# Mine268/CS-ViT

Measured on NVIDIA B200. Metric: images/sec Swin-B spatial fwd @224^2 bs256, higher is better.
Workload: dtype fp16

## Files before the change

### cs-vit_b200/csrc/mlp_fused.cu

```cuda
#include <cstdio>
#include <cstdlib>
#include <type_traits>

#include "errors.h"
#include "gemm.cuh"
#include "rowops.cuh"

namespace csvit {

constexpr uint32_t kUnit = 128 * 128;

template <int C>
struct MlpCfg {
  static constexpr int KB1 = C / 64;
  static constexpr int N2 = C / 128;
  static constexpr int NCH = 4 * C / 128;
  static constexpr int WSTAGES = 4;
  static constexpr int STG_BUFS = C == 128 ? 2 : 1;
  static constexpr uint32_t A1_BYTES = KB1 * kUnit;
  static constexpr uint32_t A2_BYTES = 2 * 2 * kUnit;
  static constexpr uint32_t W_BYTES = WSTAGES * kUnit;
  static constexpr uint32_t STG_BYTES = STG_BUFS * kEpiWarps * kStageBufBytes;
  static constexpr size_t SMEM = 1024 + size_t(A1_BYTES) + A2_BYTES + W_BYTES + STG_BYTES + 512;
};

struct MlpParams {
  const float* b1;
  int M;
  long long* trace;
};
constexpr int kMlpTraceTiles = 8;
#ifdef CSVIT_MLP_TRACE_BUILD
#define MLP_STAMP(k) do { if (tr) tr[k] = clock64(); } while (0)
#else
#define MLP_STAMP(k) do { } while (0)
#endif

constexpr int kMlpThreadsSplit = 640;
template <int FMT, int C, bool SPLIT>
__global__ void __launch_bounds__(SPLIT ? kMlpThreadsSplit : kGemmThreads, 1)
mlp_fused_kernel(const __grid_constant__ CUtensorMap tmX, const __grid_constant__ CUtensorMap tmW1,
                 const __grid_constant__ CUtensorMap tmW2, const __grid_constant__ CUtensorMap tmR, MlpParams mp, EpiParams ep) {
  using Cfg = MlpCfg<C>;
  static_assert(!SPLIT || C == 128, "the second GEMM2 accumulator fits TMEM at C = 128 only");
  constexpr int KB1 = Cfg::KB1, N2 = Cfg::N2, NCH = Cfg::NCH, WS = Cfg::WSTAGES;
  extern __shared__ uint8_t smem_raw[];
  const uint32_t base = (smem_u32(smem_raw) + 1023u) & ~1023u;
  uint8_t* smem = smem_raw + (base - smem_u32(smem_raw));
  const uint32_t a1_off = 0, a2_off = Cfg::A1_BYTES, w_off = a2_off + Cfg::A2_BYTES, stg_off = w_off + Cfg::W_BYTES;
  uint64_t* bars = reinterpret_cast<uint64_t*>(smem + stg_off + Cfg::STG_BYTES);
  uint64_t* w_full = bars;
  uint64_t* w_empty = bars + WS;
  uint64_t* acc1_full = bars + 2 * WS;
  uint64_t* acc1_empty = acc1_full + 2;
  uint64_t* a2_full = acc1_full + 4;
  uint64_t* a2_empty = acc1_full + 6;
  uint64_t* a1_full = acc1_full + 8;
  uint64_t* a1_empty = acc1_full + 9;
  uint64_t* acc2_full = acc1_full + 10;
  uint64_t* acc2_empty = acc1_full + 12;
  uint32_t* tmem_slot = reinterpret_cast<uint32_t*>(acc1_full + 14);
  uint64_t* rbar = bars + 32;

  const int warp = threadIdx.x >> 5, lane = threadIdx.x & 31;
  const int num_tiles = (mp.M + kBM - 1) / kBM;

  if (warp == 0 && lane == 0) {
    prefetch_tmap(&tmX); prefetch_tmap(&tmW1); prefetch_tmap(&tmW2);
    if (ep.tma_f32) prefetch_tmap(&tmR);
    for (int i = 0; i < 2 * kEpiWarps; ++i) mbar_init(&rbar[i], 1);
    for (int s = 0; s < WS; ++s) { mbar_init(&w_full[s], 1); mbar_init(&w_empty[s], 1); }
    for (int b = 0; b < 2; ++b) {
      mbar_init(&acc1_full[b], 1); mbar_init(&acc1_empty[b], kEpiWarps);
      mbar_init(&a2_full[b], kEpiWarps); mbar_init(&a2_empty[b], 1);
    }
    mbar_init(a1_full, 1); mbar_init(a1_empty, 1);
    for (int b = 0; b < 2; ++b) { mbar_init(&acc2_full[b], 1); mbar_init(&acc2_empty[b], kEpiWarps); }
    fence_mbar_init();
  }
  if (warp == 1) tmem_alloc(tmem_slot, 512);
  tc_fence_before();
  __syncthreads();
  tc_fence_after();
  const uint32_t tmem_base = *tmem_slot;
  griddep_launch();
  griddep_wait();
  const uint32_t tm_acc2 = tmem_base + 256;
  constexpr int EW0 = SPLIT ? 4 : 2;
  if (warp < EW0) {
  if (SPLIT) asm volatile("setmaxnreg.dec.sync.aligned.u32 64;");
  if (warp == 0) {
    if (lane == 0) {
      int s = 0; uint32_t ph = 0;
      auto load_w = [&](const CUtensorMap* tm, int col, int row) {
        mbar_wait(&w_empty[s], ph ^ 1u);
        mbar_arrive_expect_tx(&w_full[s], kUnit);
        tma_load_2d(smem + w_off + size_t(s) * kUnit, tm, &w_full[s], col, row);
        if (++s == WS) { s = 0; ph ^= 1u; }
      };
      uint32_t it = 0;
      auto load_a1 = [&](int t, uint32_t i) {
        mbar_wait(a1_empty, (i & 1u) ^ 1u);
        mbar_arrive_expect_tx(a1_full, Cfg::A1_BYTES);
        for (int kb = 0; kb < KB1; ++kb) tma_load_2d(smem + a1_off + size_t(kb) * kUnit, &tmX, a1_full, kb * 64, t * kBM);
      };
      bool pre = false;
      for (int t = blockIdx.x; t < num_tiles; t += gridDim.x, ++it) {
        if (!pre) {
          load_a1(t, it);
          for (int kb = 0; kb < KB1; ++kb) load_w(&tmW1, kb * 64, 0);
        }
        pre = false;
        for (int j = 0; j < NCH; ++j) {
          if (j + 1 < NCH) {
            for (int kb = 0; kb < KB1; ++kb) load_w(&tmW1, kb * 64, (j + 1) * 128);
          } else if (SPLIT && t + int(gridDim.x) < num_tiles) {
            load_a1(t + int(gridDim.x), it + 1);
            for (int kb = 0; kb < KB1; ++kb) load_w(&tmW1, kb * 64, 0);
            pre = true;
          }
          for (int kb2 = 0; kb2 < 2; ++kb2)
            for (int n2 = 0; n2 < N2; ++n2) load_w(&tmW2, j * 128 + kb2 * 64, n2 * 128);
        }
      }
    }
  } else if (warp == 1) {
    {
      constexpr uint32_t idesc = make_idesc(uint32_t(FMT), kBM, 128);
      int s = 0; uint32_t ph = 0;
      auto mma_unit = [&](uint32_t a_addr, uint32_t d_tmem, bool first) {
        mbar_wait(&w_full[s], ph);
        tc_fence_after();
        if (fa_elect_one()) {
          const uint64_t adesc = make_sw128_kmajor_desc(a_addr);
          const uint64_t bdesc = make_sw128_kmajor_desc(base + w_off + uint32_t(s) * kUnit);
#pragma unroll
          for (int k = 0; k < 4; ++k)
            umma_ss<false>(d_tmem, adesc + uint64_t(2 * k), bdesc + uint64_t(2 * k), idesc, (first && k == 0) ? 0u : 1u);
          umma_commit(&w_empty[s]);
        }
        __syncwarp();
        if (++s == WS) { s = 0; ph ^= 1u; }
      };
      uint32_t it = 0;
      uint32_t use[2] = {0, 0};
      auto gemm1 = [&](int j) {
        const int b = j & 1;
        mbar_wait(&acc1_empty[b], (use[b] & 1u) ^ 1u);
        tc_fence_after();
        for (int kb = 0; kb < KB1; ++kb) mma_unit(base + a1_off + uint32_t(kb) * kUnit, tmem_base + uint32_t(b * 128), kb == 0);
        if (fa_elect_one()) umma_commit(&acc1_full[b]);
        __syncwarp();
      };
      bool pre = false;
      for (int t = blockIdx.x; t < num_tiles; t += gridDim.x, ++it) {
        if (!pre) {
          mbar_wait(a1_full, it & 1u);
          tc_fence_after();
          gemm1(0);
        }
        pre = false;
        for (int j = 0; j < NCH; ++j) {
          const int b = j & 1;
          if (j + 1 < NCH) {
            gemm1(j + 1);
            if (j + 2 == NCH) { if (fa_elect_one()) umma_commit(a1_empty); __syncwarp(); }
          } else if (SPLIT && t + int(gridDim.x) < num_tiles) {
            mbar_wait(a1_full, (it + 1) & 1u);
            tc_fence_after();
            gemm1(0);
            pre = true;
          }
          mbar_wait(&a2_full[b], use[b] & 1u);
          tc_fence_after();
          const uint32_t ab = SPLIT ? (it & 1u) : 0u;
          if (j == 0) { mbar_wait(&acc2_empty[ab], ((SPLIT ? it >> 1 : it) & 1u) ^ 1u); tc_fence_after(); }
          for (int kb2 = 0; kb2 < 2; ++kb2)
            for (int n2 = 0; n2 < N2; ++n2)
              mma_unit(base + a2_off + uint32_t(b * 2 + kb2) * kUnit, tm_acc2 + ab * 128u + uint32_t(n2 * 128), j == 0 && kb2 == 0);
          if (fa_elect_one()) {
            umma_commit(&a2_empty[b]);
            if (j == NCH - 1) umma_commit(&acc2_full[ab]);
          }
          __syncwarp();
          ++use[b];
        }
      }
    }
  }
  } else if (SPLIT && warp >= 12) {
    asm volatile("setmaxnreg.dec.sync.aligned.u32 80;");
    const int e = warp - 12;
    const int quad = warp & 3;
    const int half = e >> 2;
    uint8_t* stg = smem + stg_off + e * Cfg::STG_BUFS * kStageBufBytes;
    uint32_t it = 0, rph = 0;
    for (int t = blockIdx.x; t < num_tiles; t += gridDim.x, ++it) {
      const uint32_t ab = it & 1u;
      const int row0 = t * kBM + quad * 32, colbase = half * 64;
      if (ep.red_add) {
        if (lane == 0) tma_store_wait_read0();
        __syncwarp();
      } else {
        tma_f32_prefetch<C>(ep, &tmR, stg, rbar + 2 * e, t, 0, quad, half, lane);
      }
      mbar_wait(&acc2_full[ab], (it >> 1) & 1u);
      tc_fence_after();
      const uint32_t t_addr = tm_acc2 + ab * 128u + (uint32_t(quad * 32) << 16) + uint32_t(colbase);
#pragma unroll 1
      for (int ci = 0; ci < 2; ++ci) {
        uint8_t* buf = stg + ci * kStageBufBytes;
        uint32_t rr[32];
        tmem_ld_32x32(t_addr + uint32_t(32 * ci), rr);
        tmem_ld_wait();
        if (row0 < ep.M && !ep.red_add) {
          mbar_wait(&rbar[2 * e + ci], (rph >> ci) & 1u);
          rph ^= (1u << ci);
        }
        const float4* b4 = reinterpret_cast<const float4*>(ep.bias + colbase + 32 * ci);
#pragma unroll
        for (int k = 0; k < 8; ++k) {
          float4* pp = reinterpret_cast<float4*>(buf + lane * 128 + ((k ^ (lane & 7)) << 4));
          const float4 bb = __ldg(b4 + k);
          float4 x0 = ep.red_add ? make_float4(0.f, 0.f, 0.f, 0.f) : *pp;
          x0.x += __uint_as_float(rr[4 * k]) + bb.x; x0.y += __uint_as_float(rr[4 * k + 1]) + bb.y;
          x0.z += __uint_as_float(rr[4 * k + 2]) + bb.z; x0.w += __uint_as_float(rr[4 * k + 3]) + bb.w;
          *pp = x0;
        }
        fence_proxy_async_smem();
        __syncwarp();
        if (lane == 0 && row0 < ep.M) {
          if (ep.red_add) tma_reduce_add_2d(&tmR, buf, colbase + 32 * ci, row0);
          else tma_store_2d(&tmR, buf, colbase + 32 * ci, row0);
          tma_store_commit();
        }
      }
      tc_fence_before();
      __syncwarp();
      if (lane == 0) mbar_arrive(&acc2_empty[ab]);
    }
  } else {
    if (SPLIT) asm volatile("setmaxnreg.inc.sync.aligned.u32 128;");
    const int e = warp - EW0;
    const int quad = warp & 3;
    const int half = e >> 2;
    const int r = quad * 32 + lane;
    const bool bf = FMT == 1;
    uint8_t* stg = smem + stg_off + e * Cfg::STG_BUFS * kStageBufBytes;
    uint32_t it = 0, rph = 0;
    uint32_t use[2] = {0, 0};
    for (int t = blockIdx.x; t < num_tiles; t += gridDim.x, ++it) {
      if (!SPLIT) {
        if (ep.tma_f32) tma_f32_prefetch<C>(ep, &tmR, stg, rbar + 2 * e, t, 0, quad, half, lane);
        else prefetch_resid_tile<C>(ep, t, 0, quad, half, lane);
      }
#ifdef CSVIT_MLP_TRACE_BUILD
      long long* tr = (mp.trace && blockIdx.x == 0 && e == 0 && lane == 0 && it < kMlpTraceTiles) ? mp.trace + it * 64 : nullptr;
#endif
      for (int j = 0; j < NCH; ++j) {
        const int b = j & 1;
        MLP_STAMP(4 * j);
        mbar_wait(&acc1_full[b], use[b] & 1u);
        tc_fence_after();
        MLP_STAMP(4 * j + 1);
        uint32_t rr0[32], rr1[32];
        {
          const uint32_t ta = tmem_base + (uint32_t(quad * 32) << 16) + uint32_t(b * 128 + half * 64);
          tmem_ld_32x32(ta, rr0);
          tmem_ld_32x32(ta + 32u, rr1);
          tmem_ld_wait();
        }
        tc_fence_before();
        __syncwarp();
        if (lane == 0) mbar_arrive(&acc1_empty[b]);
        uint32_t pk[32];
        epi_bias_gelu_pack32(mp.b1, bf, j * 128 + half * 64, rr0, pk);
        epi_bias_gelu_pack32(mp.b1, bf, j * 128 + half * 64 + 32, rr1, pk + 16);
        MLP_STAMP(4 * j + 2);
        mbar_wait(&a2_empty[b], (use[b] & 1u) ^ 1u);
        MLP_STAMP(4 * j + 3);
        uint8_t* dst = smem + a2_off + uint32_t(b * 2 + half) * kUnit + r * 128;
#pragma unroll
        for (int ci = 0; ci < 8; ++ci)
          *reinterpret_cast<uint4*>(dst + ((ci ^ (r & 7)) << 4)) = make_uint4(pk[4 * ci], pk[4 * ci + 1], pk[4 * ci + 2], pk[4 * ci + 3]);
        fence_proxy_async_smem();
        __syncwarp();
        if (lane == 0) mbar_arrive(&a2_full[b]);
        ++use[b];
      }
      MLP_STAMP(4 * NCH);
      if (!SPLIT) {
#ifdef CSVIT_MLP_TRACE_BUILD
        if (tr) { mbar_wait(&acc2_full[0], it & 1u); tr[4 * NCH + 1] = clock64(); }
#endif
        epilogue_tile<C>(ep, &tmR, stg, tm_acc2, &acc2_full[0], it & 1u, t, 0, quad, half, lane, 1, nullptr, &tmR, rbar + 2 * e, &rph, true);
        tc_fence_before();
        __syncwarp();
        if (lane == 0) mbar_arrive(&acc2_empty[0]);
      } else {
        MLP_STAMP(4 * NCH + 1);
      }
      MLP_STAMP(4 * NCH + 2);
    }
  }

  if (ep.tma_f32 && warp >= (SPLIT ? 12 : 2) && lane == 0) tma_store_wait_all();
  tc_fence_before();
  __syncthreads();
  if (warp == 1) tmem_dealloc(tmem_base, 512);
}

template <int FMT, int C, bool SPLIT>
static int launch_mlp_s(const CUtensorMap& tmX, const CUtensorMap& tmW1, const CUtensorMap& tmW2, const CUtensorMap& tmR,
                      const MlpParams& mp, const EpiParams& ep, cudaStream_t stream) {
  using Cfg = MlpCfg<C>;
  static DeviceOnce once;
  auto kern = mlp_fused_kernel<FMT, C, SPLIT>;
  if (once.first()) {
    CSVIT_CUDA(cudaFuncSetAttribute(kern, cudaFuncAttributeMaxDynamicSharedMemorySize, int(Cfg::SMEM)));
  }
  const int tiles = (mp.M + kBM - 1) / kBM;
  static const int cap = [] { const char* e = getenv("CSVIT_MLP_CTAS"); return e ? atoi(e) : 0; }();
  int ctas = tiles < num_sms() ? tiles : num_sms();
  if (cap > 0 && cap < ctas) ctas = cap;
  CSVIT_CUDA(launch_pdl(kern, dim3(ctas), dim3(SPLIT ? kMlpThreadsSplit : kGemmThreads), Cfg::SMEM, stream, tmX, tmW1, tmW2, tmR, mp, ep));
  return 0;
}
template <int FMT, int C>
static int launch_mlp(const CUtensorMap& tmX, const CUtensorMap& tmW1, const CUtensorMap& tmW2, const CUtensorMap& tmR,
                      const MlpParams& mp, const EpiParams& ep, cudaStream_t stream) {
  if constexpr (C == 128) {
    static const bool split = [] { const char* e = getenv("CSVIT_MLP_SPLIT"); return !(e && e[0] == '0'); }();
    if (split && ep.tma_f32 && ep.resid && ep.bias) return launch_mlp_s<FMT, C, true>(tmX, tmW1, tmW2, tmR, mp, ep, stream);
  }
  return launch_mlp_s<FMT, C, false>(tmX, tmW1, tmW2, tmR, mp, ep, stream);
}

int launch_mlp_fused(const void* xn, long long ldxn, const void* W1, long long ldw1, const float* b1, const void* W2,
                     long long ldw2, const float* b2, float* x, long long ldx, int dtype, int M, int C, cudaStream_t stream) {
  CSVIT_REQUIRE(dtype == DT_BF16 || dtype == DT_F16, "mlp_fused: 16-bit operand formats only");
  CSVIT_REQUIRE(C == 128 || C == 256, "mlp_fused: C=%d not in {128, 256}", C);
  CSVIT_REQUIRE(ldx % 4 == 0 && (reinterpret_cast<uintptr_t>(x) & 15) == 0, "mlp_fused: residual stream must be 16-byte aligned");
  if (M <= 0) return 0;
  EpiParams ep{};
  ep.bias = b2; ep.resid = x; ep.out = x; ep.ldo = ldx; ep.ldr = ldx; ep.out_dtype = DT_F32; ep.act = ACT_NONE;
  ep.M = M; ep.N = C; ep.vec_ok = 1; ep.tma_store = 0; ep.coalesced = 1;
  ep.map_mode = ROWMAP_IDENTITY; ep.geom = make_geom(1, 1, 1, 0);
  MlpParams mp{b1, M, nullptr};
#ifdef CSVIT_MLP_TRACE_BUILD
  static const char* trace_path = getenv("CSVIT_MLP_TRACE");
#else
  static const char* trace_path = nullptr;
#endif
  if (trace_path) { CSVIT_CUDA(cudaMalloc(&mp.trace, kMlpTraceTiles * 64 * sizeof(long long))); CSVIT_CUDA(cudaMemsetAsync(mp.trace, 0, kMlpTraceTiles * 64 * sizeof(long long), stream)); }
  CUtensorMap tmX, tmW1, tmW2;
  if (int e = make_tmap(&tmX, xn, ldxn, M, C, dtype, kBM, true)) return e;
  if (int e = make_tmap(&tmW1, W1, ldw1, 4ll * C, C, dtype, 128, true)) return e;
  if (int e = make_tmap(&tmW2, W2, ldw2, C, 4ll * C, dtype, 128, true)) return e;
  CUtensorMap tmR = tmX;
  static const bool tma_resid = [] { const char* e = getenv("CSVIT_MLP_TMA_RESID"); return !(e && e[0] == '0'); }();
  if (C == 128 && tma_resid && (ldx * 4) % 16 == 0) {
    ep.tma_f32 = 1; ep.coalesced = 0;
    if (int e = make_tmap(&tmR, x, ldx, M, C, DT_F32, 32, false)) return e;
  }
  static const bool split128 = [] { const char* e = getenv("CSVIT_MLP_SPLIT"); return !(e && e[0] == '0'); }();
  if (ep.tma_f32 ? red_add_mode() != 0 : red_add_mode() == 1) {
    ep.red_add = 1;
    if (!(C == 128 && ep.tma_f32 && split128)) ep.resid = nullptr;
  }
  const bool bf = dtype == DT_BF16;
  if (trace_path) {
    int e = C == 128 ? (bf ? launch_mlp<1, 128>(tmX, tmW1, tmW2, tmR, mp, ep, stream) : launch_mlp<0, 128>(tmX, tmW1, tmW2, tmR, mp, ep, stream))
                     : (bf ? launch_mlp<1, 256>(tmX, tmW1, tmW2, tmR, mp, ep, stream) : launch_mlp<0, 256>(tmX, tmW1, tmW2, tmR, mp, ep, stream));
    if (e) return e;
    CSVIT_CUDA(cudaStreamSynchronize(stream));
    long long h[kMlpTraceTiles * 64];
    CSVIT_CUDA(cudaMemcpy(h, mp.trace, sizeof(h), cudaMemcpyDeviceToHost));
    cudaFree(mp.trace);
    if (FILE* f = fopen(trace_path, "a")) {
      const int nch = 4 * C / 128;
      fprintf(f, "# mlp_fused C=%d: epilogue warp 0 of CTA 0; per chunk: wait acc1 | TMEM load + GELU | wait A2 buffer | store; then wait acc2 | residual epilogue\n", C);
      for (int t = 0; t < kMlpTraceTiles; ++t) {
        const long long* r = h + t * 64;
        if (!r[0]) continue;
        fprintf(f, "tile %d start %8lld:", t, r[0] - h[0]);
        for (int j = 0; j < nch; ++j) {
          const long long nxt = j + 1 < nch ? r[4 * j + 4] : r[4 * nch];
          fprintf(f, "  [%lld %lld %lld %lld]", r[4 * j + 1] - r[4 * j], r[4 * j + 2] - r[4 * j + 1], r[4 * j + 3] - r[4 * j + 2], nxt - r[4 * j + 3]);
        }
        fprintf(f, "  acc2 wait %lld, epilogue %lld, total %lld\n", r[4 * nch + 1] - r[4 * nch], r[4 * nch + 2] - r[4 * nch + 1], r[4 * nch + 2] - r[0]);
      }
      fclose(f);
    }
    return 0;
  }
  if (C == 128) return bf ? launch_mlp<1, 128>(tmX, tmW1, tmW2, tmR, mp, ep, stream) : launch_mlp<0, 128>(tmX, tmW1, tmW2, tmR, mp, ep, stream);
  return bf ? launch_mlp<1, 256>(tmX, tmW1, tmW2, tmR, mp, ep, stream) : launch_mlp<0, 256>(tmX, tmW1, tmW2, tmR, mp, ep, stream);
}

}
```

Baseline: 18380.

## Run fused MLP as 2-CTA cluster pairs with split weight loads

Adds a cluster-of-two variant of the fused MLP kernel that uses paired tensor-core MMAs (M=256 across two CTAs). Each CTA loads half of every weight tile, so per-CTA weight traffic and shared-memory stage size are halved, and the freed space allows more weight pipeline stages. An optional double-buffered xn input is also added. The pair path is on by default. It adds cross-CTA barrier arrivals and cluster syncs, and halves the number of independent work units.

```diff
diff --git a/cs-vit_b200/csrc/mlp_fused.cu b/cs-vit_b200/csrc/mlp_fused.cu
--- a/cs-vit_b200/csrc/mlp_fused.cu
+++ b/cs-vit_b200/csrc/mlp_fused.cu
@@ -10,18 +10,20 @@
 
 constexpr uint32_t kUnit = 128 * 128;
 
-template <int C>
+template <int C, bool PAIR = false, int XB = 1>
 struct MlpCfg {
   static constexpr int KB1 = C / 64;
   static constexpr int N2 = C / 128;
   static constexpr int NCH = 4 * C / 128;
-  static constexpr int WSTAGES = 4;
+  static constexpr uint32_t W_UNIT = PAIR ? kUnit / 2 : kUnit;
+  static constexpr int WSTAGES = PAIR && XB == 1 ? 8 : 4;
   static constexpr int STG_BUFS = C == 128 ? 2 : 1;
   static constexpr uint32_t A1_BYTES = KB1 * kUnit;
   static constexpr uint32_t A2_BYTES = 2 * 2 * kUnit;
-  static constexpr uint32_t W_BYTES = WSTAGES * kUnit;
+  static constexpr uint32_t W_BYTES = WSTAGES * W_UNIT;
   static constexpr uint32_t STG_BYTES = STG_BUFS * kEpiWarps * kStageBufBytes;
-  static constexpr size_t SMEM = 1024 + size_t(A1_BYTES) + A2_BYTES + W_BYTES + STG_BYTES + 512;
+  static constexpr size_t SMEM = 1024 + size_t(XB) * A1_BYTES + A2_BYTES + W_BYTES + STG_BYTES + 512;
+  static_assert(SMEM <= 227 * 1024, "shared memory");
 };
 
 struct MlpParams {
@@ -30,24 +32,30 @@
   long long* trace;
 };
 constexpr int kMlpTraceTiles = 8;
+constexpr int kMlpTraceIssuer = 48;
 #ifdef CSVIT_MLP_TRACE_BUILD
 #define MLP_STAMP(k) do { if (tr) tr[k] = clock64(); } while (0)
+#define MLP_TIMED_WAIT(acc, bar, par) do { const long long c0_ = clock64(); mbar_wait(bar, par); (acc) += clock64() - c0_; } while (0)
 #else
 #define MLP_STAMP(k) do { } while (0)
+#define MLP_TIMED_WAIT(acc, bar, par) mbar_wait(bar, par)
 #endif
 
 constexpr int kMlpThreadsSplit = 640;
-template <int FMT, int C, bool SPLIT>
-__global__ void __launch_bounds__(SPLIT ? kMlpThreadsSplit : kGemmThreads, 1)
-mlp_fused_kernel(const __grid_constant__ CUtensorMap tmX, const __grid_constant__ CUtensorMap tmW1,
-                 const __grid_constant__ CUtensorMap tmW2, const __grid_constant__ CUtensorMap tmR, MlpParams mp, EpiParams ep) {
-  using Cfg = MlpCfg<C>;
+
+template <int FMT, int C, bool SPLIT, bool PAIR, int XB>
+__device__ __forceinline__ void mlp_body(const CUtensorMap* tmX, const CUtensorMap* tmW1, const CUtensorMap* tmW2, const CUtensorMap* tmR,
+                                         const MlpParams& mp, const EpiParams& ep) {
+  using Cfg = MlpCfg<C, PAIR, XB>;
   static_assert(!SPLIT || C == 128, "the second GEMM2 accumulator fits TMEM at C = 128 only");
+  static_assert(XB == 1 || (XB == 2 && SPLIT), "the second xn buffer is loaded in place of the split kernel's early load");
   constexpr int KB1 = Cfg::KB1, N2 = Cfg::N2, NCH = Cfg::NCH, WS = Cfg::WSTAGES;
+  constexpr uint32_t WU = Cfg::W_UNIT;
+  constexpr uint32_t PEERS = PAIR ? 2 : 1;
   extern __shared__ uint8_t smem_raw[];
   const uint32_t base = (smem_u32(smem_raw) + 1023u) & ~1023u;
   uint8_t* smem = smem_raw + (base - smem_u32(smem_raw));
-  const uint32_t a1_off = 0, a2_off = Cfg::A1_BYTES, w_off = a2_off + Cfg::A2_BYTES, stg_off = w_off + Cfg::W_BYTES;
+  const uint32_t a1_off = 0, a2_off = XB * Cfg::A1_BYTES, w_off = a2_off + Cfg::A2_BYTES, stg_off = w_off + Cfg::W_BYTES;
   uint64_t* bars = reinterpret_cast<uint64_t*>(smem + stg_off + Cfg::STG_BYTES);
   uint64_t* w_full = bars;
   uint64_t* w_empty = bars + WS;
@@ -56,31 +64,43 @@
   uint64_t* a2_full = acc1_full + 4;
   uint64_t* a2_empty = acc1_full + 6;
   uint64_t* a1_full = acc1_full + 8;
-  uint64_t* a1_empty = acc1_full + 9;
-  uint64_t* acc2_full = acc1_full + 10;
-  uint64_t* acc2_empty = acc1_full + 12;
-  uint32_t* tmem_slot = reinterpret_cast<uint32_t*>(acc1_full + 14);
-  uint64_t* rbar = bars + 32;
+  uint64_t* a1_empty = acc1_full + 10;
+  uint64_t* acc2_full = acc1_full + 12;
+  uint64_t* acc2_empty = acc1_full + 14;
+  uint32_t* tmem_slot = reinterpret_cast<uint32_t*>(acc1_full + 16);
+  uint64_t* rbar = bars + 40;
 
   const int warp = threadIdx.x >> 5, lane = threadIdx.x & 31;
-  const int num_tiles = (mp.M + kBM - 1) / kBM;
+  const uint32_t rank = PAIR ? cluster_ctarank() : 0u;
+  const int unit0 = PAIR ? int(blockIdx.x >> 1) : int(blockIdx.x);
+  const int ustep = PAIR ? int(gridDim.x >> 1) : int(gridDim.x);
+  const int num_units = PAIR ? (mp.M + 2 * kBM - 1) / (2 * kBM) : (mp.M + kBM - 1) / kBM;
+  auto row_tile = [&](int u) { return PAIR ? 2 * u + int(rank) : u; };
+  auto arrive_issuer = [&](uint64_t* bar) {
+    if constexpr (PAIR) mbar_arrive_cluster(mapa_u32(smem_u32(bar), 0));
+    else mbar_arrive(bar);
+  };
 
   if (warp == 0 && lane == 0) {
-    prefetch_tmap(&tmX); prefetch_tmap(&tmW1); prefetch_tmap(&tmW2);
-    if (ep.tma_f32) prefetch_tmap(&tmR);
+    prefetch_tmap(tmX); prefetch_tmap(tmW1); prefetch_tmap(tmW2);
+    if (ep.tma_f32) prefetch_tmap(tmR);
     for (int i = 0; i < 2 * kEpiWarps; ++i) mbar_init(&rbar[i], 1);
-    for (int s = 0; s < WS; ++s) { mbar_init(&w_full[s], 1); mbar_init(&w_empty[s], 1); }
+    for (int s = 0; s < WS; ++s) { mbar_init(&w_full[s], PEERS); mbar_init(&w_empty[s], 1); }
     for (int b = 0; b < 2; ++b) {
-      mbar_init(&acc1_full[b], 1); mbar_init(&acc1_empty[b], kEpiWarps);
-      mbar_init(&a2_full[b], kEpiWarps); mbar_init(&a2_empty[b], 1);
-    }
-    mbar_init(a1_full, 1); mbar_init(a1_empty, 1);
-    for (int b = 0; b < 2; ++b) { mbar_init(&acc2_full[b], 1); mbar_init(&acc2_empty[b], kEpiWarps); }
+      mbar_init(&acc1_full[b], 1); mbar_init(&acc1_empty[b], PEERS * kEpiWarps);
+      mbar_init(&a2_full[b], PEERS * kEpiWarps); mbar_init(&a2_empty[b], 1);
+    }
+    for (int x = 0; x < XB; ++x) { mbar_init(&a1_full[x], PEERS); mbar_init(&a1_empty[x], 1); }
+    for (int b = 0; b < 2; ++b) { mbar_init(&acc2_full[b], 1); mbar_init(&acc2_empty[b], PEERS * kEpiWarps); }
     fence_mbar_init();
   }
-  if (warp == 1) tmem_alloc(tmem_slot, 512);
+  if (warp == 1) {
+    if constexpr (PAIR) tmem_alloc_pair(tmem_slot, 512);
+    else tmem_alloc(tmem_slot, 512);
+  }
   tc_fence_before();
   __syncthreads();
+  if constexpr (PAIR) cluster_sync_all();
   tc_fence_after();
   const uint32_t tmem_base = *tmem_slot;
   griddep_launch();
@@ -94,84 +114,116 @@
       int s = 0; uint32_t ph = 0;
       auto load_w = [&](const CUtensorMap* tm, int col, int row) {
         mbar_wait(&w_empty[s], ph ^ 1u);
-        mbar_arrive_expect_tx(&w_full[s], kUnit);
-        tma_load_2d(smem + w_off + size_t(s) * kUnit, tm, &w_full[s], col, row);
+        if constexpr (PAIR) {
+          const uint32_t lfull = mapa_u32(smem_u32(&w_full[s]), 0);
+          mbar_arrive_expect_tx_cluster(lfull, WU);
+          tma_load_2d_pair(smem + w_off + size_t(s) * WU, tm, lfull, col, row + int(rank) * 64);
+        } else {
+          mbar_arrive_expect_tx(&w_full[s], WU);
+          tma_load_2d(smem + w_off + size_t(s) * WU, tm, &w_full[s], col, row);
+        }
         if (++s == WS) { s = 0; ph ^= 1u; }
       };
+      auto load_a1 = [&](int t, uint32_t i) {
+        const uint32_t x = i % XB;
+        mbar_wait(&a1_empty[x], ((i / XB) & 1u) ^ 1u);
+        uint8_t* dst = smem + a1_off + size_t(x) * Cfg::A1_BYTES;
+        if constexpr (PAIR) {
+          const uint32_t lfull = mapa_u32(smem_u32(&a1_full[x]), 0);
+          mbar_arrive_expect_tx_cluster(lfull, Cfg::A1_BYTES);
+          for (int kb = 0; kb < KB1; ++kb) tma_load_2d_pair(dst + size_t(kb) * kUnit, tmX, lfull, kb * 64, t * kBM);
+        } else {
+          mbar_arrive_expect_tx(&a1_full[x], Cfg::A1_BYTES);
+          for (int kb = 0; kb < KB1; ++kb) tma_load_2d(dst + size_t(kb) * kUnit, tmX, &a1_full[x], kb * 64, t * kBM);
+        }
+      };
       uint32_t it = 0;
-      auto load_a1 = [&](int t, uint32_t i) {
-        mbar_wait(a1_empty, (i & 1u) ^ 1u);
-        mbar_arrive_expect_tx(a1_full, Cfg::A1_BYTES);
-        for (int kb = 0; kb < KB1; ++kb) tma_load_2d(smem + a1_off + size_t(kb) * kUnit, &tmX, a1_full, kb * 64, t * kBM);
-      };
       bool pre = false;
-      for (int t = blockIdx.x; t < num_tiles; t += gridDim.x, ++it) {
+      for (int u = unit0; u < num_units; u += ustep, ++it) {
+        const bool has_next = u + ustep < num_units;
         if (!pre) {
-          load_a1(t, it);
-          for (int kb = 0; kb < KB1; ++kb) load_w(&tmW1, kb * 64, 0);
+          load_a1(row_tile(u), it);
+          for (int kb = 0; kb < KB1; ++kb) load_w(tmW1, kb * 64, 0);
         }
         pre = false;
+        if (XB == 2 && has_next) load_a1(row_tile(u + ustep), it + 1);
         for (int j = 0; j < NCH; ++j) {
           if (j + 1 < NCH) {
-            for (int kb = 0; kb < KB1; ++kb) load_w(&tmW1, kb * 64, (j + 1) * 128);
-          } else if (SPLIT && t + int(gridDim.x) < num_tiles) {
-            load_a1(t + int(gridDim.x), it + 1);
-            for (int kb = 0; kb < KB1; ++kb) load_w(&tmW1, kb * 64, 0);
+            for (int kb = 0; kb < KB1; ++kb) load_w(tmW1, kb * 64, (j + 1) * 128);
+          } else if (SPLIT && has_next) {
+            if (XB == 1) load_a1(row_tile(u + ustep), it + 1);
+            for (int kb = 0; kb < KB1; ++kb) load_w(tmW1, kb * 64, 0);
             pre = true;
           }
           for (int kb2 = 0; kb2 < 2; ++kb2)
-            for (int n2 = 0; n2 < N2; ++n2) load_w(&tmW2, j * 128 + kb2 * 64, n2 * 128);
-        }
-      }
-    }
-  } else if (warp == 1) {
+            for (int n2 = 0; n2 < N2; ++n2) load_w(tmW2, j * 128 + kb2 * 64, n2 * 128);
+        }
+      }
+    }
+  } else if (warp == 1 && rank == 0) {
     {
-      constexpr uint32_t idesc = make_idesc(uint32_t(FMT), kBM, 128);
+      constexpr uint32_t idesc = make_idesc(uint32_t(FMT), PAIR ? 2 * kBM : kBM, 128);
+      auto commit = [&](uint64_t* bar) {
+        if constexpr (PAIR) umma_commit_pair(bar, 3);
+        else umma_commit(bar);
+      };
+#ifdef CSVIT_MLP_TRACE_BUILD
+      long long wt[3] = {0, 0, 0};
+#endif
       int s = 0; uint32_t ph = 0;
       auto mma_unit = [&](uint32_t a_addr, uint32_t d_tmem, bool first) {
-        mbar_wait(&w_full[s], ph);
+        MLP_TIMED_WAIT(wt[0], &w_full[s], ph);
         tc_fence_after();
         if (fa_elect_one()) {
           const uint64_t adesc = make_sw128_kmajor_desc(a_addr);
-          const uint64_t bdesc = make_sw128_kmajor_desc(base + w_off + uint32_t(s) * kUnit);
+          const uint64_t bdesc = make_sw128_kmajor_desc(base + w_off + uint32_t(s) * WU);
 #pragma unroll
-          for (int k = 0; k < 4; ++k)
-            umma_ss<false>(d_tmem, adesc + uint64_t(2 * k), bdesc + uint64_t(2 * k), idesc, (first && k == 0) ? 0u : 1u);
-          umma_commit(&w_empty[s]);
+          for (int k = 0; k < 4; ++k) {
+            if constexpr (PAIR) umma_ss_pair(d_tmem, adesc + uint64_t(2 * k), bdesc + uint64_t(2 * k), idesc, (first && k == 0) ? 0u : 1u);
+            else umma_ss<false>(d_tmem, adesc + uint64_t(2 * k), bdesc + uint64_t(2 * k), idesc, (first && k == 0) ? 0u : 1u);
+          }
+          commit(&w_empty[s]);
         }
         __syncwarp();
         if (++s == WS) { s = 0; ph ^= 1u; }
       };
       uint32_t it = 0;
       uint32_t use[2] = {0, 0};
-      auto gemm1 = [&](int j) {
+      auto gemm1 = [&](int j, uint32_t xb) {
         const int b = j & 1;
-        mbar_wait(&acc1_empty[b], (use[b] & 1u) ^ 1u);
+        MLP_TIMED_WAIT(wt[2], &acc1_empty[b], (use[b] & 1u) ^ 1u);
         tc_fence_after();
-        for (int kb = 0; kb < KB1; ++kb) mma_unit(base + a1_off + uint32_t(kb) * kUnit, tmem_base + uint32_t(b * 128), kb == 0);
-        if (fa_elect_one()) umma_commit(&acc1_full[b]);
+        for (int kb = 0; kb < KB1; ++kb)
+          mma_unit(base + a1_off + xb * Cfg::A1_BYTES + uint32_t(kb) * kUnit, tmem_base + uint32_t(b * 128), kb == 0);
+        if (fa_elect_one()) commit(&acc1_full[b]);
         __syncwarp();
       };
       bool pre = false;
-      for (int t = blockIdx.x; t < num_tiles; t += gridDim.x, ++it) {
+      for (int u = unit0; u < num_units; u += ustep, ++it) {
+#ifdef CSVIT_MLP_TRACE_BUILD
+        long long* itr = (mp.trace && blockIdx.x == 0 && it < kMlpTraceTiles) ? mp.trace + it * 64 + kMlpTraceIssuer : nullptr;
+        const long long t_start = clock64();
+        wt[0] = wt[1] = wt[2] = 0;
+#endif
+        const uint32_t xb = it % XB;
         if (!pre) {
-          mbar_wait(a1_full, it & 1u);
+          mbar_wait(&a1_full[xb], (it / XB) & 1u);
           tc_fence_after();
-          gemm1(0);
+          gemm1(0, xb);
         }
         pre = false;
         for (int j = 0; j < NCH; ++j) {
           const int b = j & 1;
           if (j + 1 < NCH) {
-            gemm1(j + 1);
-            if (j + 2 == NCH) { if (fa_elect_one()) umma_commit(a1_empty); __syncwarp(); }
-          } else if (SPLIT && t + int(gridDim.x) < num_tiles) {
-            mbar_wait(a1_full, (it + 1) & 1u);
+            gemm1(j + 1, xb);
+            if (j + 2 == NCH) { if (fa_elect_one()) commit(&a1_empty[xb]); __syncwarp(); }
+          } else if (SPLIT && u + ustep < num_units) {
+            mbar_wait(&a1_full[(it + 1) % XB], ((it + 1) / XB) & 1u);
             tc_fence_after();
-            gemm1(0);
+            gemm1(0, (it + 1) % XB);
             pre = true;
           }
-          mbar_wait(&a2_full[b], use[b] & 1u);
+          MLP_TIMED_WAIT(wt[1], &a2_full[b], use[b] & 1u);
           tc_fence_after();
           const uint32_t ab = SPLIT ? (it & 1u) : 0u;
           if (j == 0) { mbar_wait(&acc2_empty[ab], ((SPLIT ? it >> 1 : it) & 1u) ^ 1u); tc_fence_after(); }
@@ -179,12 +231,15 @@
             for (int n2 = 0; n2 < N2; ++n2)
               mma_unit(base + a2_off + uint32_t(b * 2 + kb2) * kUnit, tm_acc2 + ab * 128u + uint32_t(n2 * 128), j == 0 && kb2 == 0);
           if (fa_elect_one()) {
-            umma_commit(&a2_empty[b]);
-            if (j == NCH - 1) umma_commit(&acc2_full[ab]);
+            commit(&a2_empty[b]);
+            if (j == NCH - 1) commit(&acc2_full[ab]);
           }
           __syncwarp();
           ++use[b];
         }
+#ifdef CSVIT_MLP_TRACE_BUILD
+        if (itr && lane == 0) { itr[0] = wt[0]; itr[1] = wt[1]; itr[2] = wt[2]; itr[3] = clock64() - t_start; }
+#endif
       }
     }
   }
@@ -195,14 +250,15 @@
     const int half = e >> 2;
     uint8_t* stg = smem + stg_off + e * Cfg::STG_BUFS * kStageBufBytes;
     uint32_t it = 0, rph = 0;
-    for (int t = blockIdx.x; t < num_tiles; t += gridDim.x, ++it) {
+    for (int u = unit0; u < num_units; u += ustep, ++it) {
+      const int t = row_tile(u);
       const uint32_t ab = it & 1u;
       const int row0 = t * kBM + quad * 32, colbase = half * 64;
       if (ep.red_add) {
         if (lane == 0) tma_store_wait_read0();
         __syncwarp();
       } else {
-        tma_f32_prefetch<C>(ep, &tmR, stg, rbar + 2 * e, t, 0, quad, half, lane);
+        tma_f32_prefetch<C>(ep, tmR, stg, rbar + 2 * e, t, 0, quad, half, lane);
       }
       mbar_wait(&acc2_full[ab], (it >> 1) & 1u);
       tc_fence_after();
@@ -230,14 +286,14 @@
         fence_proxy_async_smem();
         __syncwarp();
         if (lane == 0 && row0 < ep.M) {
-          if (ep.red_add) tma_reduce_add_2d(&tmR, buf, colbase + 32 * ci, row0);
-          else tma_store_2d(&tmR, buf, colbase + 32 * ci, row0);
+          if (ep.red_add) tma_reduce_add_2d(tmR, buf, colbase + 32 * ci, row0);
+          else tma_store_2d(tmR, buf, colbase + 32 * ci, row0);
           tma_store_commit();
         }
       }
       tc_fence_before();
       __syncwarp();
-      if (lane == 0) mbar_arrive(&acc2_empty[ab]);
+      if (lane == 0) arrive_issuer(&acc2_empty[ab]);
     }
   } else {
     if (SPLIT) asm volatile("setmaxnreg.inc.sync.aligned.u32 128;");
@@ -249,9 +305,10 @@
     uint8_t* stg = smem + stg_off + e * Cfg::STG_BUFS * kStageBufBytes;
     uint32_t it = 0, rph = 0;
     uint32_t use[2] = {0, 0};
-    for (int t = blockIdx.x; t < num_tiles; t += gridDim.x, ++it) {
+    for (int u = unit0; u < num_units; u += ustep, ++it) {
+      const int t = row_tile(u);
       if (!SPLIT) {
-        if (ep.tma_f32) tma_f32_prefetch<C>(ep, &tmR, stg, rbar + 2 * e, t, 0, quad, half, lane);
+        if (ep.tma_f32) tma_f32_prefetch<C>(ep, tmR, stg, rbar + 2 * e, t, 0, quad, half, lane);
         else prefetch_resid_tile<C>(ep, t, 0, quad, half, lane);
       }
 #ifdef CSVIT_MLP_TRACE_BUILD
@@ -272,7 +329,7 @@
         }
         tc_fence_before();
         __syncwarp();
-        if (lane == 0) mbar_arrive(&acc1_empty[b]);
+        if (lane == 0) arrive_issuer(&acc1_empty[b]);
         uint32_t pk[32];
         epi_bias_gelu_pack32(mp.b1, bf, j * 128 + half * 64, rr0, pk);
         epi_bias_gelu_pack32(mp.b1, bf, j * 128 + half * 64 + 32, rr1, pk + 16);
@@ -285,7 +342,7 @@
           *reinterpret_cast<uint4*>(dst + ((ci ^ (r & 7)) << 4)) = make_uint4(pk[4 * ci], pk[4 * ci + 1], pk[4 * ci + 2], pk[4 * ci + 3]);
         fence_proxy_async_smem();
         __syncwarp();
-        if (lane == 0) mbar_arrive(&a2_full[b]);
+        if (lane == 0) arrive_issuer(&a2_full[b]);
         ++use[b];
       }
       MLP_STAMP(4 * NCH);
@@ -293,10 +350,10 @@
 #ifdef CSVIT_MLP_TRACE_BUILD
         if (tr) { mbar_wait(&acc2_full[0], it & 1u); tr[4 * NCH + 1] = clock64(); }
 #endif
-        epilogue_tile<C>(ep, &tmR, stg, tm_acc2, &acc2_full[0], it & 1u, t, 0, quad, half, lane, 1, nullptr, &tmR, rbar + 2 * e, &rph, true);
+        epilogue_tile<C>(ep, tmR, stg, tm_acc2, &acc2_full[0], it & 1u, t, 0, quad, half, lane, 1, nullptr, tmR, rbar + 2 * e, &rph, true);
         tc_fence_before();
         __syncwarp();
-        if (lane == 0) mbar_arrive(&acc2_empty[0]);
+        if (lane == 0) arrive_issuer(&acc2_empty[0]);
       } else {
         MLP_STAMP(4 * NCH + 1);
       }
@@ -307,33 +364,64 @@
   if (ep.tma_f32 && warp >= (SPLIT ? 12 : 2) && lane == 0) tma_store_wait_all();
   tc_fence_before();
   __syncthreads();
-  if (warp == 1) tmem_dealloc(tmem_base, 512);
+  if constexpr (PAIR) {
+    cluster_sync_all();
+    if (warp == 1) tmem_dealloc_pair(tmem_base, 512);
+  } else {
+    if (warp == 1) tmem_dealloc(tmem_base, 512);
+  }
 }
 
 template <int FMT, int C, bool SPLIT>
+__global__ void __launch_bounds__(SPLIT ? kMlpThreadsSplit : kGemmThreads, 1)
+mlp_fused_kernel(const __grid_constant__ CUtensorMap tmX, const __grid_constant__ CUtensorMap tmW1,
+                 const __grid_constant__ CUtensorMap tmW2, const __grid_constant__ CUtensorMap tmR, MlpParams mp, EpiParams ep) {
+  mlp_body<FMT, C, SPLIT, false, 1>(&tmX, &tmW1, &tmW2, &tmR, mp, ep);
+}
+
+template <int FMT, int C, bool SPLIT, int XB>
+__global__ void __cluster_dims__(2, 1, 1) __launch_bounds__(SPLIT ? kMlpThreadsSplit : kGemmThreads, 1)
+mlp_pair_kernel(const __grid_constant__ CUtensorMap tmX, const __grid_constant__ CUtensorMap tmW1,
+                const __grid_constant__ CUtensorMap tmW2, const __grid_constant__ CUtensorMap tmR, MlpParams mp, EpiParams ep) {
+  mlp_body<FMT, C, SPLIT, true, XB>(&tmX, &tmW1, &tmW2, &tmR, mp, ep);
+}
+
+template <int FMT, int C, bool SPLIT, bool PAIR, int XB>
 static int launch_mlp_s(const CUtensorMap& tmX, const CUtensorMap& tmW1, const CUtensorMap& tmW2, const CUtensorMap& tmR,
                       const MlpParams& mp, const EpiParams& ep, cudaStream_t stream) {
-  using Cfg = MlpCfg<C>;
+  using Cfg = MlpCfg<C, PAIR, XB>;
   static DeviceOnce once;
-  auto kern = mlp_fused_kernel<FMT, C, SPLIT>;
+  auto kern = [] {
+    if constexpr (PAIR) return mlp_pair_kernel<FMT, C, SPLIT, XB>;
+    else return mlp_fused_kernel<FMT, C, SPLIT>;
+  }();
   if (once.first()) {
     CSVIT_CUDA(cudaFuncSetAttribute(kern, cudaFuncAttributeMaxDynamicSharedMemorySize, int(Cfg::SMEM)));
   }
-  const int tiles = (mp.M + kBM - 1) / kBM;
+  constexpr int per = PAIR ? 2 : 1;
+  const int units = (mp.M + per * kBM - 1) / (per * kBM);
   static const int cap = [] { const char* e = getenv("CSVIT_MLP_CTAS"); return e ? atoi(e) : 0; }();
-  int ctas = tiles < num_sms() ? tiles : num_sms();
-  if (cap > 0 && cap < ctas) ctas = cap;
-  CSVIT_CUDA(launch_pdl(kern, dim3(ctas), dim3(SPLIT ? kMlpThreadsSplit : kGemmThreads), Cfg::SMEM, stream, tmX, tmW1, tmW2, tmR, mp, ep));
+  int n = units < num_sms() / per ? units : num_sms() / per;
+  if (cap > 0 && cap / per < n) n = cap / per > 0 ? cap / per : 1;
+  CSVIT_CUDA(launch_pdl(kern, dim3(n * per), dim3(SPLIT ? kMlpThreadsSplit : kGemmThreads), Cfg::SMEM, stream, tmX, tmW1, tmW2, tmR, mp, ep));
   return 0;
 }
 template <int FMT, int C>
-static int launch_mlp(const CUtensorMap& tmX, const CUtensorMap& tmW1, const CUtensorMap& tmW2, const CUtensorMap& tmR,
-                      const MlpParams& mp, const EpiParams& ep, cudaStream_t stream) {
+static int launch_mlp(const CUtensorMap& tmX, const CUtensorMap& tmW1, const CUtensorMap& tmW2, const CUtensorMap& tmW1h,
+                      const CUtensorMap& tmW2h, const CUtensorMap& tmR, const MlpParams& mp, const EpiParams& ep, cudaStream_t stream) {
+  static const bool pair = [] { const char* e = getenv("CSVIT_MLP_PAIR"); return !(e && e[0] == '0'); }();
   if constexpr (C == 128) {
     static const bool split = [] { const char* e = getenv("CSVIT_MLP_SPLIT"); return !(e && e[0] == '0'); }();
-    if (split && ep.tma_f32 && ep.resid && ep.bias) return launch_mlp_s<FMT, C, true>(tmX, tmW1, tmW2, tmR, mp, ep, stream);
-  }
-  return launch_mlp_s<FMT, C, false>(tmX, tmW1, tmW2, tmR, mp, ep, stream);
+    static const bool xn2 = [] { const char* e = getenv("CSVIT_MLP_PAIR_XN"); return e && e[0] == '2'; }();
+    if (split && ep.tma_f32 && ep.resid && ep.bias) {
+      if (pair && xn2) return launch_mlp_s<FMT, C, true, true, 2>(tmX, tmW1h, tmW2h, tmR, mp, ep, stream);
+      if (pair) return launch_mlp_s<FMT, C, true, true, 1>(tmX, tmW1h, tmW2h, tmR, mp, ep, stream);
+      return launch_mlp_s<FMT, C, true, false, 1>(tmX, tmW1, tmW2, tmR, mp, ep, stream);
+    }
+  } else {
+    if (pair) return launch_mlp_s<FMT, C, false, true, 1>(tmX, tmW1h, tmW2h, tmR, mp, ep, stream);
+  }
+  return launch_mlp_s<FMT, C, false, false, 1>(tmX, tmW1, tmW2, tmR, mp, ep, stream);
 }
 
 int launch_mlp_fused(const void* xn, long long ldxn, const void* W1, long long ldw1, const float* b1, const void* W2,
@@ -357,6 +445,9 @@
   if (int e = make_tmap(&tmX, xn, ldxn, M, C, dtype, kBM, true)) return e;
   if (int e = make_tmap(&tmW1, W1, ldw1, 4ll * C, C, dtype, 128, true)) return e;
   if (int e = make_tmap(&tmW2, W2, ldw2, C, 4ll * C, dtype, 128, true)) return e;
+  CUtensorMap tmW1h, tmW2h;
+  if (int e = make_tmap(&tmW1h, W1, ldw1, 4ll * C, C, dtype, 64, true)) return e;
+  if (int e = make_tmap(&tmW2h, W2, ldw2, C, 4ll * C, dtype, 64, true)) return e;
   CUtensorMap tmR = tmX;
   static const bool tma_resid = [] { const char* e = getenv("CSVIT_MLP_TMA_RESID"); return !(e && e[0] == '0'); }();
   if (C == 128 && tma_resid && (ldx * 4) % 16 == 0) {
@@ -370,8 +461,8 @@
   }
   const bool bf = dtype == DT_BF16;
   if (trace_path) {
-    int e = C == 128 ? (bf ? launch_mlp<1, 128>(tmX, tmW1, tmW2, tmR, mp, ep, stream) : launch_mlp<0, 128>(tmX, tmW1, tmW2, tmR, mp, ep, stream))
-                     : (bf ? launch_mlp<1, 256>(tmX, tmW1, tmW2, tmR, mp, ep, stream) : launch_mlp<0, 256>(tmX, tmW1, tmW2, tmR, mp, ep, stream));
+    int e = C == 128 ? (bf ? launch_mlp<1, 128>(tmX, tmW1, tmW2, tmW1h, tmW2h, tmR, mp, ep, stream) : launch_mlp<0, 128>(tmX, tmW1, tmW2, tmW1h, tmW2h, tmR, mp, ep, stream))
+                     : (bf ? launch_mlp<1, 256>(tmX, tmW1, tmW2, tmW1h, tmW2h, tmR, mp, ep, stream) : launch_mlp<0, 256>(tmX, tmW1, tmW2, tmW1h, tmW2h, tmR, mp, ep, stream));
     if (e) return e;
     CSVIT_CUDA(cudaStreamSynchronize(stream));
     long long h[kMlpTraceTiles * 64];
@@ -379,7 +470,10 @@
     cudaFree(mp.trace);
     if (FILE* f = fopen(trace_path, "a")) {
       const int nch = 4 * C / 128;
-      fprintf(f, "# mlp_fused C=%d: epilogue warp 0 of CTA 0; per chunk: wait acc1 | TMEM load + GELU | wait A2 buffer | store; then wait acc2 | residual epilogue\n", C);
+      static const bool pair = [] { const char* e = getenv("CSVIT_MLP_PAIR"); return !(e && e[0] == '0'); }();
+      fprintf(f, "# mlp_fused C=%d M=%d (%s kernel): epilogue warp 0 of CTA 0; per chunk: wait acc1 | TMEM load + GELU | wait A2 buffer | store; "
+                 "then wait acc2 | residual epilogue; issuer of CTA 0 per tile: cycles waiting on w_full (weights), a2_full (GELU chunk), acc1_empty, "
+                 "and the tile's issue span\n", C, M, pair ? "pair" : "single-CTA");
       for (int t = 0; t < kMlpTraceTiles; ++t) {
         const long long* r = h + t * 64;
         if (!r[0]) continue;
@@ -389,13 +483,15 @@
           fprintf(f, "  [%lld %lld %lld %lld]", r[4 * j + 1] - r[4 * j], r[4 * j + 2] - r[4 * j + 1], r[4 * j + 3] - r[4 * j + 2], nxt - r[4 * j + 3]);
         }
         fprintf(f, "  acc2 wait %lld, epilogue %lld, total %lld\n", r[4 * nch + 1] - r[4 * nch], r[4 * nch + 2] - r[4 * nch + 1], r[4 * nch + 2] - r[0]);
+        const long long* q = r + kMlpTraceIssuer;
+        fprintf(f, "    issuer: w_full wait %lld, a2_full wait %lld, acc1_empty wait %lld, span %lld\n", q[0], q[1], q[2], q[3]);
       }
       fclose(f);
     }
     return 0;
   }
-  if (C == 128) return bf ? launch_mlp<1, 128>(tmX, tmW1, tmW2, tmR, mp, ep, stream) : launch_mlp<0, 128>(tmX, tmW1, tmW2, tmR, mp, ep, stream);
-  return bf ? launch_mlp<1, 256>(tmX, tmW1, tmW2, tmR, mp, ep, stream) : launch_mlp<0, 256>(tmX, tmW1, tmW2, tmR, mp, ep, stream);
-}
-
-}
+  if (C == 128) return bf ? launch_mlp<1, 128>(tmX, tmW1, tmW2, tmW1h, tmW2h, tmR, mp, ep, stream) : launch_mlp<0, 128>(tmX, tmW1, tmW2, tmW1h, tmW2h, tmR, mp, ep, stream);
+  return bf ? launch_mlp<1, 256>(tmX, tmW1, tmW2, tmW1h, tmW2h, tmR, mp, ep, stream) : launch_mlp<0, 256>(tmX, tmW1, tmW2, tmW1h, tmW2h, tmR, mp, ep, stream);
+}
+
+}
```

Result: no change. 18480 (median of 6 runs) (+0.6%).
